# thu-uav/Multi-UAV-pursuit-evasion

Hardware: AMD Instinct MI355X
Metric: env agent-steps/sec at 65536 envs, HideAndSeek 3v1; 1/2/4/8 GPU (higher is better)
Workload: dtype f32

## Files before the change

multi-uav-pursuit-evasion_amd/csrc/hns_common.h:

```cpp
#pragma once
#include <hip/hip_runtime.h>

#include <cstdint>

#include "hns_device.h"

namespace hns {

constexpr int kEPB = 64;
constexpr int kMaxK = 4;
constexpr int kWideK = 16;
__host__ __device__ constexpr int red_stride(int NT) { return NT == 2 ? 11 : 9; }
enum { R_AERR = 0, R_TD, R_DIST, R_SPEED, R_CC, R_CD, R_CW, R_COLL,
       R_SMOOTH = R_AERR, R_FLAGS = R_TD,
       R_FX = R_DIST, R_FY = R_SPEED, R_FZ = R_CC,
       R_TWX = R_CD,
       R_F1X = 8,
       R_CPOS = R_DIST, R_CVEL = R_DIST + 3 };
enum { F_CAP = 1, F_BLOCKED = 2, F_DET = 4, F_DET1 = 8 };
constexpr int kGridStride = 516;
constexpr int kSmallWgPerCu = 2;
constexpr int kMaxT = 2;

template <int A>
struct Geo {
    static constexpr int NA = kEPB * A;
    static constexpr int T = kEPB * (A + 1);
};

struct Params {
    hns_cfg cfg;
    hns_buffers buf;
    const float *action;
    const uint8_t *reset_mask;
    uint32_t seed_lo, seed_hi, epoch;
    unsigned long long *prof;
    uint32_t cyl_magic;
    float *tasks;
    int32_t task_first;
    uint32_t prio_boost;
};

struct StepArgs {
    const float *action;
    float *prev_action, *drone_state, *pid_integ, *pid_last_rate, *throttle;
    const void *aux;
    const Params *rest;
};
static_assert(sizeof(StepArgs) == 64, "the argument block of the step kernel is sized for the fast launch path");
#define HNS_STEP_PARAMS                                                                                                                    \
    const Params *ka_rest, const float *ka_action, float *ka_prev_action, float *ka_drone_state, const void *ka_aux, float *ka_pid_integ, \
        float *ka_pid_last_rate, float *ka_throttle
#define HNS_STEP_ARGS_PACK const StepArgs ka{ka_action, ka_prev_action, ka_drone_state, ka_pid_integ, ka_pid_last_rate, ka_throttle, ka_aux, ka_rest}

HNS_DEV void warm_params(const Params *rest) {
    typedef const uint32_t __attribute__((address_space(4))) WordC;
    WordC *w = (WordC *)rest;
    uint32_t acc = 0;
#pragma unroll
    for (int i = 0; i < (int)((sizeof(Params) + 63) / 64); ++i) acc |= w[i * 16];
    asm volatile("" : : "s"(acc));
}

constexpr int kProfSlots = 16;
HNS_DEV void prof_mark(unsigned long long *prof, int slot) {
    if (prof && (threadIdx.x & 63) == 0) {
        int wave = blockIdx.x * (blockDim.x >> 6) + (threadIdx.x >> 6);
        prof[(size_t)wave * kProfSlots + slot] = (slot >= 14) ? __builtin_amdgcn_s_memrealtime() : __builtin_readcyclecounter();
#ifdef HNS_PROF_HWID
        if (slot == 0) prof[(size_t)wave * kProfSlots + 13] = __builtin_amdgcn_s_getreg(63492);
#endif
    }
}

struct Lds {
    int ds, cyl, cyl_stride, tp, red, ocyl, total;
};
__host__ __device__ inline int slab_floats(int A, int K, int NT);
__host__ __device__ inline int r4(int n) { return (n + 3) & ~3; }
__host__ __device__ constexpr int slab_rows(int A) { return A > 4 ? 32 : 64; }
__host__ __device__ inline int slab_floats(int A, int K, int NT) {
    const int rows = slab_rows(A);
    int m = rows * (NT == 2 ? 24 : HNS_SELF_DIM);
    if (K > kMaxK) K = 0;
    if (rows * K * 5 > m) m = rows * K * 5;
    if (rows * (A - 1) * 3 > m) m = rows * (A - 1) * 3;
    return r4(m);
}
__host__ __device__ inline Lds lds_layout(int A, int C, int K, int NT = 1) {
    Lds L;
    int o = 0;
    L.ds = o;    o += r4(kEPB * A * 13);
    L.cyl_stride = (3 * C) | 1;
    L.cyl = o;   o += r4(kEPB * L.cyl_stride);
    L.tp = o;    o += r4(kEPB * 3 * NT);
    L.red = o;   o += r4(kEPB * A * red_stride(NT));
    const int rows = K > kMaxK ? 0 : kEPB * A * K * 5, slabs = A * slab_floats(A, K, NT);
    L.ocyl = o;  o += r4(rows > slabs ? rows : slabs);
    L.total = o;
    return L;
}

template <int T>
HNS_DEV void coop_g2s(float *__restrict__ dst, const float *__restrict__ src, int n) {
    const int n4 = ((reinterpret_cast<uintptr_t>(src) & 15) == 0) ? (n >> 2) : 0;
    const float4 *s4 = reinterpret_cast<const float4 *>(src);
    float4 *d4 = reinterpret_cast<float4 *>(dst);
    for (int i = threadIdx.x; i < n4; i += T) d4[i] = s4[i];
    for (int i = (n4 << 2) + threadIdx.x; i < n; i += T) dst[i] = src[i];
}
template <int T>
HNS_DEV void coop_s2g(float *__restrict__ dst, const float *__restrict__ src, int n) {
    const int n4 = ((reinterpret_cast<uintptr_t>(dst) & 15) == 0) ? (n >> 2) : 0;
    const float4 *s4 = reinterpret_cast<const float4 *>(src);
    float4 *d4 = reinterpret_cast<float4 *>(dst);
    for (int i = threadIdx.x; i < n4; i += T) d4[i] = s4[i];
    for (int i = (n4 << 2) + threadIdx.x; i < n; i += T) dst[i] = src[i];
}
template <int T, int N>
HNS_DEV void coop_copy_full(float *__restrict__ dst, const float *__restrict__ src) {
    static_assert(N % 4 == 0, "float4 granularity");
    constexpr int N4 = N / 4;
    const float4 *s4 = reinterpret_cast<const float4 *>(src) + threadIdx.x;
    float4 *d4 = reinterpret_cast<float4 *>(dst) + threadIdx.x;
#pragma unroll
    for (int k = 0; k < (N4 + T - 1) / T; ++k)
        if (k * T + (int)threadIdx.x < N4) d4[k * T] = s4[k * T];
}
template <int T>
HNS_DEV void coop_s2g_masked(float *__restrict__ dst, const float *__restrict__ src, int n, int per_env,
                             const uint8_t *__restrict__ smask) {
    for (int i = threadIdx.x; i < n; i += T)
        if (smask[i / per_env]) dst[i] = src[i];
}
template <int T, bool TO_LDS>
HNS_DEV void coop_cyl(float *__restrict__ lds, float *__restrict__ g, int nenv, int c3, int stride, unsigned magic,
                      const uint8_t *__restrict__ smask) {
    for (int i = threadIdx.x; i < nenv * c3; i += T) {
        int le = (int)__umulhi((unsigned)i, magic), j = i - le * c3;
        if (TO_LDS) lds[le * stride + j] = g[i];
        else if (smask[le]) g[i] = lds[le * stride + j];
    }
}
HNS_DEV bool rigid_not_finite(const Rigid &s) {
    float a = s.pos.x;
    a = a + s.pos.y; a = a + s.pos.z; a = a + s.q.w; a = a + s.q.x; a = a + s.q.y; a = a + s.q.z;
    a = a + s.lin.x; a = a + s.lin.y; a = a + s.lin.z; a = a + s.ang.x; a = a + s.ang.y; a = a + s.ang.z;
    return (a - a) != 0.0f;
}
HNS_DEV void flag_nonfinite(uint32_t *word, bool bad, uint32_t bit) {
    if (word && bad) atomicOr(word, bit);
}
HNS_DEV void load_rigid(const float *r, Rigid &s) {
    s.pos = {r[0], r[1], r[2]};
    s.q = {r[3], r[4], r[5], r[6]};
    s.lin = {r[7], r[8], r[9]};
    s.ang = {r[10], r[11], r[12]};
}
HNS_DEV void store_rigid(float *r, const Rigid &s) {
    r[0] = s.pos.x; r[1] = s.pos.y; r[2] = s.pos.z;
    r[3] = s.q.w; r[4] = s.q.x; r[5] = s.q.y; r[6] = s.q.z;
    r[7] = s.lin.x; r[8] = s.lin.y; r[9] = s.lin.z;
    r[10] = s.ang.x; r[11] = s.ang.y; r[12] = s.ang.z;
}

HNS_DEV void st_f4(float4 *p, const float4 &v) {
    typedef float f4 __attribute__((ext_vector_type(4)));
    const f4 x = {v.x, v.y, v.z, v.w};
    asm volatile("global_store_dwordx4 %0, %1, off sc1\n\ts_nop 1" : : "v"(p), "v"(x) : "memory");
}
HNS_DEV void st_f1(float *p, float v) {
    asm volatile("global_store_dword %0, %1, off sc1\n\ts_nop 0" : : "v"(p), "v"(v) : "memory");
}

template <int NF, int ROWS = 64>
HNS_DEV void wave_store_rows(float *__restrict__ slab, float *__restrict__ gslice, const float (&row)[NF], int lane, int valid_rows = 64) {
    static_assert(ROWS == 64 || ROWS == 32, "whole wave or half a wave per pass");
    const uintptr_t gaddr = reinterpret_cast<uintptr_t>(gslice);
    const uintptr_t guni = ((uintptr_t)(uint32_t)__builtin_amdgcn_readfirstlane((int)(uint32_t)(gaddr >> 32)) << 32) |
                           (uintptr_t)(uint32_t)__builtin_amdgcn_readfirstlane((int)(uint32_t)gaddr);
    const int vrows = __builtin_amdgcn_readfirstlane(valid_rows);
#pragma unroll
    for (int half = 0; half < 64 / ROWS; ++half) {
        if (ROWS == 64 || (lane >> 5) == half) {
            float *mine = slab + (lane & (ROWS - 1)) * NF;
            if constexpr (NF % 4 == 0) {
#pragma unroll
                for (int i = 0; i < NF / 4; ++i) reinterpret_cast<float4 *>(mine)[i] = make_float4(row[4 * i], row[4 * i + 1], row[4 * i + 2], row[4 * i + 3]);
            } else if constexpr (NF % 2 == 0) {
#pragma unroll
                for (int i = 0; i < NF / 2; ++i) reinterpret_cast<float2 *>(mine)[i] = make_float2(row[2 * i], row[2 * i + 1]);
            } else {
#pragma unroll
                for (int i = 0; i < NF; ++i) mine[i] = row[i];
            }
        }
        __builtin_amdgcn_fence(__ATOMIC_RELEASE, "wavefront");
        __builtin_amdgcn_wave_barrier();
        constexpr int N4 = ROWS * NF / 4;
        const float4 *s4 = reinterpret_cast<const float4 *>(slab) + lane;
        typedef unsigned u4 __attribute__((ext_vector_type(4)));
        int rows_here = vrows - half * ROWS;
        rows_here = rows_here < 0 ? 0 : (rows_here > ROWS ? ROWS : rows_here);
        const __amdgpu_buffer_rsrc_t rs = __builtin_amdgcn_make_buffer_rsrc(reinterpret_cast<void *>(guni + (uintptr_t)half * ROWS * NF * 4), 0, rows_here * NF * 4, 0x00020000);
#pragma unroll
        for (int j = 0; j < (N4 + 63) / 64; ++j)
            if (j * 64 + lane < N4) {
                const float4 v = s4[j * 64];
                __builtin_amdgcn_raw_buffer_store_b128((u4){__float_as_uint(v.x), __float_as_uint(v.y), __float_as_uint(v.z), __float_as_uint(v.w)}, rs,
                                                       (j * 64 + lane) * 16, 0, 16 );
            }
        __builtin_amdgcn_fence(__ATOMIC_ACQUIRE, "wavefront");
        __builtin_amdgcn_wave_barrier();
    }
}

template <int NT, bool LOS, int KM = kMaxK, int KT = KM + 1, class Cfg>
HNS_DEV void cylinder_pass(const Cfg &c, int C, int K, const V3 &pos, const V3 &tp, const V3 &tpB, const float *cyl,
                           int bi[KM + 1], bool &any_block, bool &any_block1) {
    static_assert(KT >= 2 && KT <= KM + 1, "tracked keys");
    constexpr int kTrack = KT;
    uint32_t key[kTrack];
#pragma unroll
    for (int i = 0; i < kTrack; ++i) key[i] = 0x7F80000Fu;
    LosLine los = {}, los1 = {};
    if constexpr (LOS) los = d_los_setup(c, pos, tp);
    bool los_uncertain = false, los_uncertain1 = false;
    float mb0 = kInf, mt0 = kInf, mb1 = kInf, mt1 = kInf;
    any_block = false; any_block1 = false;
    if constexpr (LOS && NT == 2) los1 = d_los_setup(c, pos, tpB);
#pragma unroll 4
    for (int k = 0; k < C; ++k) {
        const float ccx = cyl[3 * k], ccy = cyl[3 * k + 1], ccz = cyl[3 * k + 2];
        const float ex = pos.x - ccx, ey = pos.y - ccy, ez = pos.z - ccz;
        if constexpr (LOS) any_block = d_los_cylinder_fast_acc(los, ccx, ccy, ccz, ex, ey, mb0, mt0) || any_block;
        if constexpr (LOS && NT == 2) any_block1 = d_los_cylinder_fast_acc(los1, ccx, ccy, ccz, ex, ey, mb1, mt1) || any_block1;
        const float d2 = HNS_FMA(ez, ez, HNS_FMA(ey, ey, ex * ex));
        uint32_t nk = (__float_as_uint(d2) & 0xFFFFFFF0u) | (uint32_t)k;
#pragma unroll
        for (int i = 0; i < kTrack; ++i) {
            uint32_t lo = min(key[i], nk);
            nk = max(key[i], nk);
            key[i] = lo;
        }
    }
    if constexpr (LOS) {
        los_uncertain = d_los_uncertain(los, mb0, mt0);
        if constexpr (NT == 2) los_uncertain1 = d_los_uncertain(los1, mb1, mt1);
        if (los_uncertain) any_block = d_blocked_exact(c, C, los, cyl);
        if (NT == 2 && los_uncertain1) any_block1 = d_blocked_exact(c, C, los1, cyl);
    }
    float bd[kTrack];
#pragma unroll
    for (int i = 0; i < kTrack; ++i) { bd[i] = __uint_as_float(key[i] & 0xFFFFFFF0u); bi[i] = (int)(key[i] & 15u); }
    bool order_safe = bd[0] > 1e-5f;
#pragma unroll
    for (int i = 0; i < kTrack - 1; ++i)
        if (i < K) order_safe = order_safe && (bd[i + 1] > bd[i] * 1.0000152587890625f);
    if (!order_safe) {
        if (!(__builtin_isfinite(pos.x) && __builtin_isfinite(pos.y) && __builtin_isfinite(pos.z))) {
#pragma unroll
            for (int i = 0; i < kTrack; ++i) bi[i] = i < C ? i : 0;
            return;
        }
#pragma unroll
        for (int i = 0; i < kTrack; ++i) { bd[i] = kInf; bi[i] = 0; }
        for (int k = 0; k < C; ++k) {
            float md = d_norm3(pos.x - cyl[3 * k], pos.y - cyl[3 * k + 1], pos.z - cyl[3 * k + 2]) - c.cylinder_size;
            if (md < bd[kTrack - 2]) {
                bd[kTrack - 2] = md; bi[kTrack - 2] = k;
#pragma unroll
                for (int i = kTrack - 2; i > 0; --i) {
                    if (bd[i] < bd[i - 1]) {
                        float td = bd[i]; bd[i] = bd[i - 1]; bd[i - 1] = td;
                        int ti = bi[i]; bi[i] = bi[i - 1]; bi[i - 1] = ti;
                    }
                }
            }
        }
    }
}

template <int A, int NT, bool STAGED = false, int PS = 13, int KM = kMaxK, class Cfg = hns_cfg>
HNS_DEV void agent_obs(const Cfg &c, int C, int K, int le, int a, const Rigid &s, const V3 &tp, const V3 &tpB, float progress,
                       const float *cyl, const float *sDS, float *gOth, float *sOCyl, float *gSelf, float *gState,
                       bool &blocked, bool &det, bool &blockedB, bool &detB, int knn_idx[KM], bool knn_masked[KM], bool st = true, bool st_oth = true,
                       float *gOCyl = nullptr, float *dist_out = nullptr, bool st_ocyl = true) {
    static_assert(!(STAGED && KM > kMaxK), "wide k-nearest selections are not staged");
    constexpr int SDW = NT == 2 ? 24 : HNS_SELF_DIM;
    const int lane = threadIdx.x & 63;
    float rtx = s.pos.x - tp.x, rty = s.pos.y - tp.y, rtz = s.pos.z - tp.z;
    float dist = d_norm3(rtx, rty, rtz);
    if (dist_out) *dist_out = dist;
    const float t = progress * c.inv_max_episode_length;
    V3 heading = d_quat_rot_x(s.q);
    V3 up = d_quat_rot_z(s.q, 1.0f);
    float4 v0 = make_float4(rtx, rty, rtz, s.q.w);
    float4 v1 = make_float4(s.q.x, s.q.y, s.q.z, s.lin.x);
    float4 v2 = make_float4(s.lin.y, s.lin.z, heading.x, heading.y);
    float4 v3 = make_float4(heading.z, up.x, up.y, up.z);
    float4 v4 = make_float4(t, t, t, t);
    float4 *so = reinterpret_cast<float4 *>(gSelf);
    if constexpr (!STAGED) {
        if (st) { so[0] = v0; so[1] = v1; so[2] = v2; so[3] = v3; so[4] = v4; }
        if (gState && st) {
            float4 *ss = reinterpret_cast<float4 *>(gState);
            ss[0] = v0; ss[1] = v1; ss[2] = v2; ss[3] = v3; ss[4] = v4;
        }
    }
    float dist1 = 0.0f;
    float4 v5 = make_float4(0, 0, 0, 0);
    if constexpr (NT == 2) {
        const float r1x = s.pos.x - tpB.x, r1y = s.pos.y - tpB.y, r1z = s.pos.z - tpB.z;
        dist1 = d_norm3(r1x, r1y, r1z);
        v5 = make_float4(r1x, r1y, r1z, 0.0f);
        if constexpr (!STAGED) {
            if (st) so[5] = v5;
            if (gState && st) reinterpret_cast<float4 *>(gState)[5] = v5;
        }
    }
    if constexpr (STAGED) {
        float row[SDW] = {v0.x, v0.y, v0.z, v0.w, v1.x, v1.y, v1.z, v1.w, v2.x, v2.y, v2.z, v2.w, v3.x, v3.y, v3.z, v3.w, v4.x, v4.y, v4.z, v4.w};
        if constexpr (NT == 2) { row[20] = v5.x; row[21] = v5.y; row[22] = v5.z; row[23] = v5.w; }
        if (st) wave_store_rows<SDW, slab_rows(A)>(sOCyl, gSelf - lane * SDW, row, lane);
        if (gState && st) wave_store_rows<SDW, slab_rows(A)>(sOCyl, gState - lane * SDW, row, lane);
    }
    if (A > 1) {
        float o[(A > 1 ? A - 1 : 1) * 3];
#pragma unroll
        for (int w = 0; w < A - 1; ++w) {
            const int j = w + (w >= a ? 1 : 0);
            const float *rj = sDS + (le * A + j) * PS;
            o[3 * w] = s.pos.x - rj[0]; o[3 * w + 1] = s.pos.y - rj[1]; o[3 * w + 2] = s.pos.z - rj[2];
        }
        if constexpr (STAGED) {
            if (st_oth) wave_store_rows<(A > 1 ? A - 1 : 1) * 3, slab_rows(A)>(sOCyl, gOth - lane * (A - 1) * 3, o, lane);
        } else if (!st_oth) {
        } else if ((((A - 1) * 3) & 1) == 0) {
            float2 *g2 = reinterpret_cast<float2 *>(gOth);
#pragma unroll
            for (int i = 0; i < (A - 1) * 3 / 2; ++i) g2[i] = make_float2(o[2 * i], o[2 * i + 1]);
        } else {
#pragma unroll
            for (int i = 0; i < (A - 1) * 3; ++i) gOth[i] = o[i];
        }
    }
    int bi[KM + 1];
    bool any_block, any_block1;
    cylinder_pass<NT, true, KM>(c, C, K, s.pos, tp, tpB, cyl, bi, any_block, any_block1);
    blocked = any_block;
    det = (dist < c.drone_detect_radius) && !blocked;
    if constexpr (NT == 2) {
        blockedB = any_block1;
        detB = (dist1 < c.drone_detect_radius) && !any_block1;
    }
    float *oc = KM > kMaxK ? gOCyl : sOCyl + (le * A + a) * K * 5;
    float krow[STAGED ? kMaxK * 5 : 1];
#pragma unroll
    for (int sidx = 0; sidx < KM; ++sidx) {
        if (sidx < K) {
            const float *cc = cyl + 3 * bi[sidx];
            bool masked = cc[2] < 0.0f;
            knn_idx[sidx] = bi[sidx];
            knn_masked[sidx] = masked;
            float *row = STAGED ? krow + sidx * 5 : oc + sidx * 5;
            const float mv = c.mask_value, ch = c.cylinder_height, cs = c.cylinder_size;
            row[0] = masked ? mv : s.pos.x - cc[0];
            row[1] = masked ? mv : s.pos.y - cc[1];
            row[2] = masked ? mv : s.pos.z - cc[2];
            row[3] = masked ? mv : ch;
            row[4] = masked ? mv : cs;
        }
    }
    if constexpr (STAGED) {
        if (st_ocyl) {
            if (K == 3) {
                float r[15];
#pragma unroll
                for (int i = 0; i < 15; ++i) r[i] = krow[i];
                wave_store_rows<15, slab_rows(A)>(sOCyl, gOCyl - lane * 15, r, lane);
            } else if (K == 4) {
                wave_store_rows<20, slab_rows(A)>(sOCyl, gOCyl - lane * 20, krow, lane);
            } else if (K == 2) {
                float r[10];
#pragma unroll
                for (int i = 0; i < 10; ++i) r[i] = krow[i];
                wave_store_rows<10, slab_rows(A)>(sOCyl, gOCyl - lane * 10, r, lane);
            } else {
                float r[5];
#pragma unroll
                for (int i = 0; i < 5; ++i) r[i] = krow[i];
                wave_store_rows<5, slab_rows(A)>(sOCyl, gOCyl - lane * 5, r, lane);
            }
        }
    }
}

}
```

multi-uav-pursuit-evasion_amd/csrc/hns_step_body.inc:

```
    HNS_STEP_ARGS_PACK;
    static_assert(GEN || KM == kMaxK, "wide k-nearest selections: the generic instantiation");
    static_assert(!MOTOR || GEN, "motor-command input: the generic instantiation");
    static_assert(CS == 0 || (!GEN && !PROF && CS <= HNS_MAX_CYLINDERS), "fixed shapes: the tuned instantiation only");
    typedef const Params __attribute__((address_space(4))) ParamsC;
    ParamsC &p = *(ParamsC *)ka.rest;
    constexpr int NA = Geo<A>::NA, SD = NT == 2 ? 24 : HNS_SELF_DIM, kRedS = red_stride(NT), T3 = 3 * NT;
    extern __shared__ __align__(16) float smem[];
    const auto &c = p.cfg;
    const auto &b = p.buf;
    const int tid = threadIdx.x, lane = tid & 63;
    const int e0 = blockIdx.x * kEPB;
    int nv = kEPB, Etot = 0;
    if constexpr (GEN) { Etot = c.num_envs; nv = Etot - e0 < kEPB ? Etot - e0 : kEPB; }
    if (tid < NA) {
        const int le = tid / A, a = tid - le * A;
        const unsigned ia = (unsigned)e0 * A + tid;
        const bool valid = !GEN || le < nv;
        const int vrows = GEN ? nv * A - (tid & ~63) : 64;
        const unsigned il = GEN ? (unsigned)(e0 + (le < nv ? le : nv - 1)) * A + a : ia;
        const float4 act4 = reinterpret_cast<const float4 *>(ka.action)[il];
        float4 prev4 = make_float4(0.f, 0.f, 0.f, 0.f);
        if constexpr (!MOTOR) prev4 = reinterpret_cast<const float4 *>(ka.prev_action)[il];
        constexpr int N4 = 64 * 13 / 4;
        const float4 *rows4 = reinterpret_cast<const float4 *>(ka.drone_state + ((size_t)e0 * A + (tid & ~63)) * 13) + lane;
        static_assert(N4 > 192 && N4 <= 256, "three full passes and a partial one");
        float4 rr0 = make_float4(0.f, 0.f, 0.f, 0.f), rr1 = rr0, rr2 = rr0, rr3 = rr0;
        if constexpr (!GEN) {
            rr0 = rows4[0]; rr1 = rows4[64]; rr2 = rows4[128];
            if (lane < N4 - 192) rr3 = rows4[192];
        }
        float4 integ4 = make_float4(0.f, 0.f, 0.f, 0.f);
        if constexpr (NT == 1 && !MOTOR) integ4 = reinterpret_cast<const float4 *>(ka.pid_integ)[il];
        float4 last4 = make_float4(0.f, 0.f, 0.f, 0.f);
        if constexpr (MOTOR) last4.w = ka.pid_last_rate[(size_t)il * 4 + 3];
        else last4 = reinterpret_cast<const float4 *>(ka.pid_last_rate)[il];
        unsigned rp = 0;
        if constexpr (NT == 1) {
            const uint8_t *rpp = static_cast<const uint8_t *>(ka.aux);
            const uint8_t *rsafe = rpp ? rpp : reinterpret_cast<const uint8_t *>(ka.action);
            const unsigned byte = rsafe[GEN ? (e0 + (le < nv ? le : nv - 1)) : (e0 + le)];
            rp = rpp ? byte : 0u;
        }
        float4 thr4 = reinterpret_cast<const float4 *>(ka.throttle)[il];
        constexpr int kStage = NT == 2 ? (3 * HNS_MAX_CYLINDERS + A - 1) / A : 1, kOwnCyl = NT == 2 ? (HNS_MAX_CYLINDERS + A - 1) / A : 1;
        float stage_v[kStage], own_c[kOwnCyl][3];
        if constexpr (NT == 2) {
            const uintptr_t cw = reinterpret_cast<uintptr_t>(ka.aux);
            const int Cq = CS ? CS : (int)(cw & 15) + 1;
            typedef const float __attribute__((address_space(1))) gcf;
            const gcf *cyl0 = reinterpret_cast<const gcf *>(cw & ~(uintptr_t)15);
            const gcf *gc = cyl0 + (size_t)e0 * Cq * 3 + lane;
#pragma unroll
            for (int i = 0; i < kStage; ++i) {
                const int pass = (tid >> 6) + i * A;
                stage_v[i] = (pass < 3 * Cq && (!GEN || pass * 64 + lane < nv * 3 * Cq)) ? gc[pass * 64] : 0.0f;
            }
            const gcf *gcy = cyl0 + (size_t)(e0 + (GEN && le >= nv ? nv - 1 : le)) * Cq * 3;
#pragma unroll
            for (int i = 0; i < kOwnCyl; ++i) {
                const int k = a + i * A;
                const int kc = k < Cq ? k : 0;
                own_c[i][0] = gcy[3 * kc]; own_c[i][1] = gcy[3 * kc + 1]; own_c[i][2] = gcy[3 * kc + 2];
            }
            if constexpr (!MOTOR) integ4 = reinterpret_cast<const float4 *>(ka.pid_integ)[il];
        }
        __builtin_amdgcn_sched_barrier(0);
        if constexpr (PROF) prof_mark(p.prof, 0);
        if constexpr (PROF) prof_mark(p.prof, 14);
        const int C = CS ? CS : c.num_cylinders, K = CS ? 3 : c.obs_max_cylinder;
        const bool with_state = c.write_critic_state && b.state_drones != nullptr;
        const LdsV3 L = lds_layout_v3(A, C, K, NT);
        float *sPub = smem + L.pub, *sCyl = smem + L.cyl, *sTp = smem + L.tp, *sRed = smem + L.red;
        float *slab = smem + L.slab + (tid >> 6) * L.slab_stride;
        V3 etp0 = {0.f, 0.f, 0.f}, etp1 = {0.f, 0.f, 0.f};
        if constexpr (NT == 2) {
            {
                const uint8_t *rsafe = b.reset_pid ? b.reset_pid : reinterpret_cast<const uint8_t *>(ka.action);
                const unsigned byte = rsafe[e0 + (GEN && le >= nv ? nv - 1 : le)];
                rp = b.reset_pid ? byte : 0u;
            }
            const float *gt = b.target_pos + (size_t)(e0 + (GEN && le >= nv ? nv - 1 : le)) * T3;
            etp0 = V3{gt[0], gt[1], gt[2]};
            etp1 = V3{gt[3], gt[4], gt[5]};
        }
        float4 ta = act4;
        if constexpr (!MOTOR) ta = d_action_tanh(act4);
        Rigid s;
        if constexpr (GEN) {
            load_rigid(ka.drone_state + (size_t)il * 13, s);
        } else {
            float4 *s4 = reinterpret_cast<float4 *>(slab) + lane;
            s4[0] = rr0; s4[64] = rr1; s4[128] = rr2;
            if (lane < N4 - 192) s4[192] = rr3;
            __builtin_amdgcn_fence(__ATOMIC_RELEASE, "wavefront");
            __builtin_amdgcn_wave_barrier();
            load_rigid(slab + lane * 13, s);
            __builtin_amdgcn_fence(__ATOMIC_ACQUIRE, "wavefront");
            __builtin_amdgcn_wave_barrier();
        }
        if constexpr (PROF) prof_mark(p.prof, 1);
        const bool boost = p.prio_boost != 0;
        if (boost) __builtin_amdgcn_s_setprio(1);
        const float los_t = last4.w;
        float cmd[4], thr_diff, aerr, thrust[4], moment[4];
        float ctbr4[4], trate[3];
        if constexpr (MOTOR) {
            cmd[0] = ta.x; cmd[1] = ta.y; cmd[2] = ta.z; cmd[3] = ta.w;
            aerr = b.action_error[il];
        } else {
        {
            const bool r = rp != 0;
            integ4.x = r ? 0.0f : integ4.x; integ4.y = r ? 0.0f : integ4.y; integ4.z = r ? 0.0f : integ4.z;
            last4.x = r ? 0.0f : last4.x; last4.y = r ? 0.0f : last4.y; last4.z = r ? 0.0f : last4.z;
        }
        d_ctbr_pid_squashed(c, ta, s.q, s.ang, prev4, integ4, last4, cmd, aerr, ctbr4, trate);
        asm volatile("" : "+v"(thr4.x), "+v"(thr4.y), "+v"(thr4.z), "+v"(thr4.w));
        if (b.ctbr && valid) reinterpret_cast<float4 *>(b.ctbr)[ia] = make_float4(ctbr4[0], ctbr4[1], ctbr4[2], ctbr4[3]);
        if (b.target_rate && valid) reinterpret_cast<float4 *>(b.target_rate)[ia] = make_float4(trate[0], trate[1], trate[2], 0.0f);
        }
        d_rotor(c, cmd, thr4, thrust, moment, thr_diff);
        const float ts = ((thrust[0] + thrust[1]) + thrust[2]) + thrust[3];
        const V3 tw = d_quat_rot_z(s.q, ts);
        const float inv_ntw = d_downwash_inv_norm(tw);
        {
            float *pub = sPub + tid * kPub;
            pub[0] = s.pos.x; pub[1] = s.pos.y; pub[2] = s.pos.z;
            pub[3] = tw.x; pub[4] = tw.y; pub[5] = tw.z;
            pub[9] = inv_ntw;
            pub[10] = los_t;
            float *red = sRed + tid * kRedS;
            red[R_AERR] = aerr; red[R_TD] = thr_diff;
            if constexpr (NT == 2) {
                const int los = (int)los_t;
                const V3 f0 = d_prey_pursuer_term(c, s.pos, etp0, (los & 1) != 0);
                const V3 f1 = d_prey_pursuer_term(c, s.pos, etp1, (los & 2) != 0);
                red[R_FX] = f0.x; red[R_FY] = f0.y; red[R_FZ] = f0.z;
                red[R_F1X] = f1.x; red[R_F1X + 1] = f1.y; red[R_F1X + 2] = f1.z;
                float *term = smem + L.term + le * L.term_stride;
#pragma unroll
                for (int i = 0; i < kOwnCyl; ++i) {
                    const int k = a + i * A;
                    if (k < C) {
                        float tx, ty;
                        d_prey_cylinder_term(c, etp1, own_c[i][0], own_c[i][1], own_c[i][2], tx, ty);
                        term[2 * k] = tx; term[2 * k + 1] = ty;
                    }
                }
                const int c3 = 3 * C;
#pragma unroll
                for (int i = 0; i < kStage; ++i) {
                    const int pass = (tid >> 6) + i * A;
                    if (pass < c3) {
                        const int idx = pass * 64 + lane;
                        const int row = (int)__umulhi((unsigned)idx, p.cyl_magic), col = idx - row * c3;
                        sCyl[row * L.cyl_stride + col] = stage_v[i];
                    }
                }
            }
        }
        if constexpr (PROF) prof_mark(p.prof, 2);
        __syncthreads();
        if constexpr (PROF) prof_mark(p.prof, 12);
        V3 fdw = {0.f, 0.f, 0.f};
#pragma unroll
        for (int o = 0; o < A - 1; ++o) {
            const int j = o + (o >= a ? 1 : 0);
            const float *pj = sPub + (le * A + j) * kPub;
            const V3 posj = {pj[0], pj[1], pj[2]}, twj = {pj[3], pj[4], pj[5]};
            const V3 fj = d_downwash_pair(s.pos, posj, twj, pj[9]);
            fdw.x = (o == 0) ? fj.x : fdw.x + fj.x;
            fdw.y = (o == 0) ? fj.y : fdw.y + fj.y;
            fdw.z = (o == 0) ? fj.z : fdw.z + fj.z;
        }
        const V3 fw = {tw.x + fdw.x, tw.y + fdw.y, tw.z + fdw.z};
        V3 tb;
        tb.x = ((c.rotor_py[0] * thrust[0] + c.rotor_py[1] * thrust[1]) + c.rotor_py[2] * thrust[2]) + c.rotor_py[3] * thrust[3];
        tb.y = -(((c.rotor_px[0] * thrust[0] + c.rotor_px[1] * thrust[1]) + c.rotor_px[2] * thrust[2]) + c.rotor_px[3] * thrust[3]);
        tb.z = ((moment[0] + moment[1]) + moment[2]) + moment[3];
        d_integrate(c, s, fw, tb);
        if constexpr (CONTACT) {
            float *red = sRed + tid * kRedS;
            red[R_CPOS] = s.pos.x; red[R_CPOS + 1] = s.pos.y; red[R_CPOS + 2] = s.pos.z;
            red[R_CVEL] = s.lin.x; red[R_CVEL + 1] = s.lin.y; red[R_CVEL + 2] = s.lin.z;
        } else {
            flag_nonfinite(b.nonfinite, valid && rigid_not_finite(s), 1u);
            float *pub = sPub + tid * kPub;
            pub[6] = s.pos.x; pub[7] = s.pos.y; pub[8] = s.pos.z;
        }
        if (valid) {
            st_f4(reinterpret_cast<float4 *>(b.throttle) + ia, thr4);
            if constexpr (!MOTOR) {
                st_f4(reinterpret_cast<float4 *>(b.pid_integ) + ia, integ4);
                st_f4(reinterpret_cast<float4 *>(b.prev_action) + ia, prev4);
                st_f1(b.action_error + ia, aerr);
            }
        }
        if constexpr (CONTACT) {
            __syncthreads();
            const float *cyl = sCyl + le * L.cyl_stride;
            d_contact_step<A, CS>(c, s, a, sRed + le * A * kRedS, cyl, C);
            flag_nonfinite(b.nonfinite, valid && rigid_not_finite(s), 1u);
            float *pub = sPub + tid * kPub;
            pub[6] = s.pos.x; pub[7] = s.pos.y; pub[8] = s.pos.z;
        }
        {
            const float row[13] = {s.pos.x, s.pos.y, s.pos.z, s.q.w, s.q.x, s.q.y, s.q.z, s.lin.x, s.lin.y, s.lin.z, s.ang.x, s.ang.y, s.ang.z};
            wave_store_rows<13>(slab, b.drone_state + ((size_t)e0 * A + (tid & ~63)) * 13, row, lane, vrows);
        }
        if constexpr (PROF) prof_mark(p.prof, 3);
        __syncthreads();
        if constexpr (PROF) prof_mark(p.prof, 8);
        if (boost) __builtin_amdgcn_s_setprio(0);
        const float progress = sTp[kEPB * T3 + le];
        const V3 tp = {sTp[le * T3], sTp[le * T3 + 1], sTp[le * T3 + 2]};
        V3 tpB = tp;
        if constexpr (NT == 2) tpB = V3{sTp[le * T3 + 3], sTp[le * T3 + 4], sTp[le * T3 + 5]};
        const float *cyl = sCyl + le * L.cyl_stride;
        const float rtx = s.pos.x - tp.x, rty = s.pos.y - tp.y, rtz = s.pos.z - tp.z;
        const float d = d_norm3(rtx, rty, rtz);
        int knn_idx[KM + 1];
        bool knn_masked[KM];
        bool blocked, blockedB;
        cylinder_pass<NT, true, KM, (CS ? 4 : KM + 1)>(c, C, K, s.pos, tp, tpB, cyl, knn_idx, blocked, blockedB);
        const bool det = (d < c.drone_detect_radius) && !blocked;
        last4.w = (float)((blocked ? 1 : 0) + (NT == 2 && blockedB ? 2 : 0));
        if constexpr (MOTOR) { if (valid) b.pid_last_rate[(size_t)ia * 4 + 3] = last4.w; }
        else if (valid) reinterpret_cast<float4 *>(b.pid_last_rate)[ia] = last4;
#pragma unroll
        for (int sidx = 0; sidx < KM; ++sidx) knn_masked[sidx] = (sidx < K) ? cyl[3 * knn_idx[sidx] + 2] < 0.0f : false;
        if constexpr (PROF) prof_mark(p.prof, 9);
        bool cap_ok = (d < c.catch_radius) && !blocked, all_blk = blocked, detB = false;
        float dn = d;
        float r1x = 0.f, r1y = 0.f, r1z = 0.f;
        if constexpr (NT == 2) {
            r1x = s.pos.x - tpB.x; r1y = s.pos.y - tpB.y; r1z = s.pos.z - tpB.z;
            const float d1 = d_norm3(r1x, r1y, r1z);
            detB = (d1 < c.drone_detect_radius) && !blockedB;
            cap_ok = cap_ok || ((d1 < c.catch_radius) && !blockedB);
            all_blk = blocked && blockedB;
            dn = d1 < d ? d1 : d;
        }
        const float act = (dn > c.catch_radius) ? 1.0f : 0.0f;
        const float dist_rew = (-c.dist_reward_coef * dn) * act;
        bool fast = false;
        {
            const float sp2 = HNS_FMA(s.lin.z, s.lin.z, HNS_FMA(s.lin.y, s.lin.y, s.lin.x * s.lin.x));
            const float v2 = c.v_drone * c.v_drone;
            fast = sp2 > v2 * 1.00000190734863f;
            if (!fast && !(sp2 < v2 * 0.99999809265137f)) fast = __builtin_sqrtf(sp2) > c.v_drone;
        }
        const float speed_rew = -c.speed_coef * (fast ? 1.0f : 0.0f);
        float cc = 0.f, cd = 0.f;
        const float rc = c.cylinder_size + c.collision_radius, rc2 = rc * rc;
#pragma unroll
        for (int sidx = 0; sidx < KM; ++sidx) {
            if (sidx < K) {
                const float *cy = cyl + 3 * knn_idx[sidx];
                const float rx = s.pos.x - cy[0], ry = s.pos.y - cy[1];
                const float s2 = HNS_FMA(ry, ry, rx * rx);
                bool h = s2 < rc2 * 0.99999618530273f;
                if (!h && !(s2 > rc2 * 1.00000381469727f)) h = (__builtin_sqrtf(s2) - c.cylinder_size) < c.collision_radius;
                float hit = h ? 1.0f : 0.0f;
                if (knn_masked[sidx]) hit = 0.0f;
                cc = (sidx == 0) ? hit : cc + hit;
            }
        }
        float cr = -c.collision_coef * cc;
        const float dd2 = c.coll_drone_dist * c.coll_drone_dist;
#pragma unroll
        for (int o = 0; o < A - 1; ++o) {
            const int j = o + (o >= a ? 1 : 0);
            const float *rj = sPub + (le * A + j) * kPub + 6;
            const float ex = s.pos.x - rj[0], ey = s.pos.y - rj[1], ez = s.pos.z - rj[2];
            const float s3 = HNS_FMA(ez, ez, HNS_FMA(ey, ey, ex * ex));
            bool h = s3 < dd2 * 0.99999809265137f;
            if (!h && !(s3 > dd2 * 1.00000190734863f)) h = __builtin_sqrtf(s3) < c.coll_drone_dist;
            const float hit = h ? 1.0f : 0.0f;
            cd = (o == 0) ? hit : cd + hit;
        }
        cr = cr + -c.collision_coef * cd;
        const float cw = ((s.pos.z > c.max_height) ? 1.0f : 0.0f) + ((HNS_FMA(s.pos.y, s.pos.y, s.pos.x * s.pos.x) > c.arena_sq) ? 1.0f : 0.0f);
        cr = cr + -c.collision_coef * cw;
        float sm = 0.0f;
        if (c.use_deployment) sm = c.smoothness_coef * d_expf(-aerr);
        {
            float *red = sRed + tid * kRedS;
            red[R_DIST] = dist_rew; red[R_SPEED] = speed_rew; red[R_CC] = cc; red[R_CD] = cd; red[R_CW] = cw;
            red[R_COLL] = cr; red[R_SMOOTH] = sm;
            red[R_FLAGS] = __int_as_float((cap_ok ? F_CAP : 0) | (all_blk ? F_BLOCKED : 0) | (det ? F_DET : 0) | (detB ? F_DET1 : 0));
        }
        if constexpr (PROF) prof_mark(p.prof, 4);
        __syncthreads();
        if constexpr (PROF) prof_mark(p.prof, 5);
        bool det_any = false, det_any1 = false;
#pragma unroll
        for (int j = 0; j < A; ++j) {
            const int fl = __float_as_int(sRed[(le * A + j) * kRedS + R_FLAGS]);
            det_any |= (fl & F_DET) != 0;
            det_any1 |= (fl & F_DET1) != 0;
        }
        {
            const float t = progress * c.inv_max_episode_length;
            const V3 heading = d_quat_rot_x(s.q), up = d_quat_rot_z(s.q, 1.0f);
            const float m = c.mask_value;
            float row[SD] = {det_any ? rtx : m, det_any ? rty : m, det_any ? rtz : m, s.q.w, s.q.x, s.q.y, s.q.z, s.lin.x, s.lin.y, s.lin.z,
                             heading.x, heading.y, heading.z, up.x, up.y, up.z, t, t, t, t};
            if constexpr (NT == 2) { row[20] = det_any1 ? r1x : m; row[21] = det_any1 ? r1y : m; row[22] = det_any1 ? r1z : m; row[23] = 0.0f; }
            wave_store_rows<SD, slab_rows_v4(A, NT)>(slab, b.obs_self + ((size_t)e0 * A + (tid & ~63)) * SD, row, lane, vrows);
            if (with_state) {
                float rs[SD];
#pragma unroll
                for (int i = 0; i < SD; ++i) rs[i] = row[i];
                rs[0] = rtx; rs[1] = rty; rs[2] = rtz;
                if constexpr (NT == 2) { rs[20] = r1x; rs[21] = r1y; rs[22] = r1z; }
                wave_store_rows<SD, slab_rows_v4(A, NT)>(slab, b.state_drones + ((size_t)e0 * A + (tid & ~63)) * SD, rs, lane, vrows);
            }
        }
        if constexpr (A > 1) {
            float o[(A > 1 ? A - 1 : 1) * 3];
#pragma unroll
            for (int w = 0; w < A - 1; ++w) {
                const int j = w + (w >= a ? 1 : 0);
                const float *rj = sPub + (le * A + j) * kPub + 6;
                o[3 * w] = s.pos.x - rj[0]; o[3 * w + 1] = s.pos.y - rj[1]; o[3 * w + 2] = s.pos.z - rj[2];
            }
            wave_store_rows<(A > 1 ? A - 1 : 1) * 3, slab_rows_v4(A, NT)>(slab, b.obs_others + ((size_t)e0 * A + (tid & ~63)) * (A - 1) * 3, o, lane, vrows);
        }
        if constexpr (KM > kMaxK) {
            const float mv = c.mask_value, ch = c.cylinder_height, cs = c.cylinder_size;
            float *oc = b.obs_cylinders + (size_t)ia * K * 5;
            if (valid) {
#pragma unroll
                for (int sidx = 0; sidx < KM; ++sidx) {
                    if (sidx < K) {
                        const float *cc = cyl + 3 * knn_idx[sidx];
                        const bool masked = knn_masked[sidx];
                        oc[sidx * 5] = masked ? mv : s.pos.x - cc[0];
                        oc[sidx * 5 + 1] = masked ? mv : s.pos.y - cc[1];
                        oc[sidx * 5 + 2] = masked ? mv : s.pos.z - cc[2];
                        oc[sidx * 5 + 3] = masked ? mv : ch;
                        oc[sidx * 5 + 4] = masked ? mv : cs;
                    }
                }
            }
        } else {
            float krow[kMaxK * 5];
            const float mv = c.mask_value, ch = c.cylinder_height, cs = c.cylinder_size;
#pragma unroll
            for (int sidx = 0; sidx < kMaxK; ++sidx) {
                const float *cc = cyl + 3 * ((sidx < K) ? knn_idx[sidx] : 0);
                const bool masked = knn_masked[sidx];
                const float rx = s.pos.x - cc[0], ry = s.pos.y - cc[1], rz = s.pos.z - cc[2];
                krow[sidx * 5] = masked ? mv : rx;
                krow[sidx * 5 + 1] = masked ? mv : ry;
                krow[sidx * 5 + 2] = masked ? mv : rz;
                krow[sidx * 5 + 3] = masked ? mv : ch;
                krow[sidx * 5 + 4] = masked ? mv : cs;
            }
            float *g = b.obs_cylinders + ((size_t)e0 * A + (tid & ~63)) * K * 5;
            if (K == 3) {
                float r[15];
#pragma unroll
                for (int i = 0; i < 15; ++i) r[i] = krow[i];
                wave_store_rows<15, slab_rows_v4(A, NT)>(slab, g, r, lane, vrows);
            } else if (K == 4) {
                wave_store_rows<20, slab_rows_v4(A, NT)>(slab, g, krow, lane, vrows);
            } else if (K == 2) {
                float r[10];
#pragma unroll
                for (int i = 0; i < 10; ++i) r[i] = krow[i];
                wave_store_rows<10, slab_rows_v4(A, NT)>(slab, g, r, lane, vrows);
            } else {
                float r[5];
#pragma unroll
                for (int i = 0; i < 5; ++i) r[i] = krow[i];
                wave_store_rows<5, slab_rows_v4(A, NT)>(slab, g, r, lane, vrows);
            }
        }
        if constexpr (PROF) prof_mark(p.prof, 6);
    } else {
        __builtin_amdgcn_s_setprio(2);
        const int le = lane;
        const bool valid = !GEN || le < nv;
        const int e = e0 + (valid ? le : nv - 1);
#ifndef HNS_NO_WARM
        warm_params(ka.rest);
#endif
        if constexpr (PROF) prof_mark(p.prof, 0);
        if constexpr (PROF) prof_mark(p.prof, 14);
        const int C = CS ? CS : c.num_cylinders, K = CS ? 3 : c.obs_max_cylinder, E = c.stats_stride;
        const LdsV3 L = lds_layout_v3(A, C, K, NT);
        float *sPub = smem + L.pub, *sCyl = smem + L.cyl, *sTp = smem + L.tp, *sRed = smem + L.red, *sEnvOut = smem + L.envout;
        float *cylw = sCyl + le * L.cyl_stride;
        const float *gt = b.target_pos + (size_t)e * T3;
        const V3 tp0 = {gt[0], gt[1], gt[2]};
        V3 tp1 = tp0;
        if constexpr (NT == 2) tp1 = V3{gt[3], gt[4], gt[5]};
        float progress = b.progress[e];
        if constexpr (NT == 1 && GEN) {
            const float *gr = b.cylinders + (size_t)e * C * 3;
            for (int j = 0; j < 3 * C; ++j) cylw[j] = gr[j];
            __builtin_amdgcn_fence(__ATOMIC_RELEASE, "wavefront");
            __builtin_amdgcn_wave_barrier();
        } else if constexpr (NT == 1) {
            const float *gc = b.cylinders + (size_t)e0 * C * 3 + lane;
            const int c3 = 3 * C;
            int i0 = 0;
            for (; i0 + 24 <= c3; i0 += 24) {
                float cv[24];
#pragma unroll
                for (int i = 0; i < 24; ++i) cv[i] = gc[(i0 + i) * 64];
#pragma unroll
                for (int i = 0; i < 24; ++i) {
                    const int idx = (i0 + i) * 64 + lane;
                    const int row = (int)__umulhi((unsigned)idx, p.cyl_magic), col = idx - row * c3;
                    sCyl[row * L.cyl_stride + col] = cv[i];
                }
            }
            for (; i0 < c3; i0 += 3) {
                float cv[3];
#pragma unroll
                for (int i = 0; i < 3; ++i) cv[i] = gc[(i0 + i) * 64];
#pragma unroll
                for (int i = 0; i < 3; ++i) {
                    const int idx = (i0 + i) * 64 + lane;
                    const int row = (int)__umulhi((unsigned)idx, p.cyl_magic), col = idx - row * c3;
                    sCyl[row * L.cyl_stride + col] = cv[i];
                }
            }
            __builtin_amdgcn_fence(__ATOMIC_RELEASE, "wavefront");
            __builtin_amdgcn_wave_barrier();
        }
        progress += 1.0f;
        sTp[kEPB * T3 + le] = progress;
        if constexpr (PROF) prof_mark(p.prof, 1);
        float st[HNS_NUM_STATS];
        if constexpr (NT == 1) {
#pragma unroll
            for (int i = 0; i < HNS_NUM_STATS; ++i) st[i] = b.stats[(size_t)i * E + e];
        }
        bool out_of_arena = false;
        const V3 Fenv = d_prey_arena_term(c, tp0, out_of_arena);
        float fcx = 0.f, fcy = 0.f;
        if constexpr (NT == 2) {
            const float *cylg = b.cylinders + (size_t)e * C * 3;
            if ((C & 3) == 0) {
                const float4 *g4 = reinterpret_cast<const float4 *>(cylg);
                for (int k0 = 0; k0 < C; k0 += 4) {
                    const float4 q0 = g4[3 * (k0 >> 2)], q1 = g4[3 * (k0 >> 2) + 1], q2 = g4[3 * (k0 >> 2) + 2];
                    const float v[12] = {q0.x, q0.y, q0.z, q0.w, q1.x, q1.y, q1.z, q1.w, q2.x, q2.y, q2.z, q2.w};
#pragma unroll
                    for (int i = 0; i < 4; ++i) {
                        float tx, ty;
                        d_prey_cylinder_term(c, tp0, v[3 * i], v[3 * i + 1], v[3 * i + 2], tx, ty);
                        fcx += tx;
                        fcy += ty;
                    }
                }
            } else {
                for (int k = 0; k < C; ++k) {
                    float tx, ty;
                    d_prey_cylinder_term(c, tp0, cylg[3 * k], cylg[3 * k + 1], cylg[3 * k + 2], tx, ty);
                    fcx += tx;
                    fcy += ty;
                }
            }
        } else {
#pragma unroll 4
            for (int k = 0; k < C; ++k) {
                float tx, ty;
                d_prey_cylinder_term(c, tp0, cylw[3 * k], cylw[3 * k + 1], cylw[3 * k + 2], tx, ty);
                fcx += tx;
                fcy += ty;
            }
        }
        V3 Fenv1 = {0.f, 0.f, 0.f};
        float gcx = 0.f, gcy = 0.f;
        if constexpr (NT == 2) {
            bool out1 = false;
            Fenv1 = d_prey_arena_term(c, tp1, out1);
            out_of_arena = out_of_arena || out1;
#pragma unroll
            for (int i = 0; i < HNS_NUM_STATS; ++i) st[i] = b.stats[(size_t)i * E + e];
        }
        if constexpr (PROF) prof_mark(p.prof, 2);
        __syncthreads();
        if constexpr (PROF) prof_mark(p.prof, 12);
#ifndef HNS_NO_PIN
#pragma unroll
        for (int i = 0; i < HNS_NUM_STATS; ++i) asm volatile("" : "+v"(st[i]));
#endif
        V3 F = {0.f, 0.f, 0.f}, G = {0.f, 0.f, 0.f};
#pragma unroll
        for (int j = 0; j < A; ++j) {
            if constexpr (NT == 2) {
                const float *red = sRed + (le * A + j) * kRedS;
                F.x = (j == 0) ? red[R_FX] : F.x + red[R_FX];
                F.y = (j == 0) ? red[R_FY] : F.y + red[R_FY];
                F.z = (j == 0) ? red[R_FZ] : F.z + red[R_FZ];
                G.x = (j == 0) ? red[R_F1X] : G.x + red[R_F1X];
                G.y = (j == 0) ? red[R_F1X + 1] : G.y + red[R_F1X + 1];
                G.z = (j == 0) ? red[R_F1X + 2] : G.z + red[R_F1X + 2];
            } else {
                const float *pj = sPub + (le * A + j) * kPub;
                const V3 dp = {pj[0], pj[1], pj[2]};
                const int los = (int)pj[10];
                const V3 fp = d_prey_pursuer_term(c, dp, tp0, (los & 1) != 0);
                F.x = (j == 0) ? fp.x : F.x + fp.x;
                F.y = (j == 0) ? fp.y : F.y + fp.y;
                F.z = (j == 0) ? fp.z : F.z + fp.z;
            }
        }
        if constexpr (NT == 2) {
            const float *term = smem + L.term + le * L.term_stride;
#pragma unroll 4
            for (int k = 0; k < C; ++k) {
                gcx += term[2 * k];
                gcy += term[2 * k + 1];
            }
        }
        F.x = F.x + Fenv.x; F.y = F.y + Fenv.y; F.z = F.z + Fenv.z;
        F.x = F.x + fcx; F.y = F.y + fcy; F.z = F.z + 0.0f;
        const V3 tvel = {(c.v_prey * F.x) / (__builtin_fabsf(F.x) + 1e-5f), (c.v_prey * F.y) / (__builtin_fabsf(F.y) + 1e-5f),
                         (c.v_prey * F.z) / (__builtin_fabsf(F.z) + 1e-5f)};
        V3 tpn = {tp0.x + tvel.x * c.dt, tp0.y + tvel.y * c.dt, tp0.z + tvel.z * c.dt};
        if constexpr (CONTACT) {
            float vx = 0.0f, vy = 0.0f;
            d_contact_cylinders<false, CS>(tpn, vx, vy, cylw, C, c.contact_rt, c.contact_rt2, c.cylinder_height);
        }
        sTp[le * T3] = tpn.x; sTp[le * T3 + 1] = tpn.y; sTp[le * T3 + 2] = tpn.z;
        { const float sf = (tpn.x + tpn.y) + tpn.z; flag_nonfinite(b.nonfinite, valid && (sf - sf) != 0.0f, 2u); }
        V3 tvel1 = {0.f, 0.f, 0.f};
        if constexpr (NT == 2) {
            G.x = G.x + Fenv1.x; G.y = G.y + Fenv1.y; G.z = G.z + Fenv1.z;
            G.x = G.x + gcx; G.y = G.y + gcy; G.z = G.z + 0.0f;
            tvel1 = V3{(c.v_prey * G.x) / (__builtin_fabsf(G.x) + 1e-5f), (c.v_prey * G.y) / (__builtin_fabsf(G.y) + 1e-5f),
                       (c.v_prey * G.z) / (__builtin_fabsf(G.z) + 1e-5f)};
            const V3 tpn1 = {tp1.x + tvel1.x * c.dt, tp1.y + tvel1.y * c.dt, tp1.z + tvel1.z * c.dt};
            sTp[le * T3 + 3] = tpn1.x; sTp[le * T3 + 4] = tpn1.y; sTp[le * T3 + 5] = tpn1.z;
            { const float sf = (tpn1.x + tpn1.y) + tpn1.z; flag_nonfinite(b.nonfinite, valid && (sf - sf) != 0.0f, 2u); }
        }
        {
            sEnvOut[le * T3] = tvel.x; sEnvOut[le * T3 + 1] = tvel.y; sEnvOut[le * T3 + 2] = tvel.z;
            if constexpr (NT == 2) { sEnvOut[le * T3 + 3] = tvel1.x; sEnvOut[le * T3 + 4] = tvel1.y; sEnvOut[le * T3 + 5] = tvel1.z; }
            env_store_slice<GEN>(sTp, b.target_pos + (size_t)e0 * T3, kEPB * T3, lane, nv * T3);
            env_store_slice<GEN>(sEnvOut, b.target_vel + (size_t)e0 * T3, kEPB * T3, lane, nv * T3);
        }
        if constexpr (CONTACT) __syncthreads();
        {
            float sum_ae = 0.f, sum_td = 0.f, max_td = 0.f;
#pragma unroll
            for (int j = 0; j < A; ++j) {
                const float *red = sRed + (le * A + j) * kRedS;
                const float td = red[R_TD];
                sum_ae = (j == 0) ? red[R_AERR] : sum_ae + red[R_AERR];
                sum_td = (j == 0) ? td : sum_td + td;
                max_td = (j == 0) ? td : (td > max_td ? td : max_td);
            }
            const float mae = sum_ae * c.inv_num_agents;
            st[HNS_ST_ACTION_ERROR_ORDER1_MEAN] += mae;
            if (mae > st[HNS_ST_ACTION_ERROR_ORDER1_MAX]) st[HNS_ST_ACTION_ERROR_ORDER1_MAX] = mae;
            st[HNS_ST_OUT_OF_ARENA] = ((st[HNS_ST_OUT_OF_ARENA] != 0.0f) || out_of_arena) ? 1.0f : 0.0f;
            st[HNS_ST_SMOOTHNESS_COEF] = c.smoothness_coef;
            st[HNS_ST_SMOOTHNESS_MEAN] += sum_td * c.inv_num_agents;
            if (max_td > st[HNS_ST_SMOOTHNESS_MAX]) st[HNS_ST_SMOOTHNESS_MAX] = max_td;
        }
        if constexpr (PROF) prof_mark(p.prof, 3);
        __syncthreads();
        if constexpr (PROF) prof_mark(p.prof, 8);
        if constexpr (PROF) prof_mark(p.prof, 4);
        __syncthreads();
        if constexpr (PROF) prof_mark(p.prof, 5);
        const float iA = c.inv_num_agents;
        bool any_cap = false, all_blocked = true, any_coll = false, det_any = false, det_any1 = false;
        float sum_dist = 0, sum_speed = 0, sum_cc = 0, sum_cd = 0, sum_cw = 0, sum_coll = 0, sum_smooth = 0;
#pragma unroll
        for (int j = 0; j < A; ++j) {
            const float *red = sRed + (le * A + j) * kRedS;
            const int fl = __float_as_int(red[R_FLAGS]);
            any_cap |= (fl & F_CAP) != 0;
            all_blocked &= (fl & F_BLOCKED) != 0;
            det_any |= (fl & F_DET) != 0;
            det_any1 |= (fl & F_DET1) != 0;
            any_coll |= red[R_COLL] < 0.0f;
            if (j == 0) {
                sum_dist = red[R_DIST]; sum_speed = red[R_SPEED]; sum_cc = red[R_CC]; sum_cd = red[R_CD]; sum_cw = red[R_CW];
                sum_coll = red[R_COLL]; sum_smooth = red[R_SMOOTH];
            } else {
                sum_dist += red[R_DIST]; sum_speed += red[R_SPEED]; sum_cc += red[R_CC]; sum_cd += red[R_CD]; sum_cw += red[R_CW];
                sum_coll += red[R_COLL]; sum_smooth += red[R_SMOOTH];
            }
        }
        const float detf = (det_any || (NT == 2 && det_any1)) ? 1.0f : 0.0f;
        const float detect_rew = c.detect_reward_coef * detf;
        const float catch_rew = c.catch_reward_coef * (any_cap ? 1.0f : 0.0f);
        float sum_rew = 0.f;
#pragma unroll
        for (int j = 0; j < A; ++j) {
            const float *red = sRed + (le * A + j) * kRedS;
            const float r = ((((red[R_DIST] + detect_rew) + catch_rew) + red[R_COLL]) + red[R_SPEED]) + red[R_SMOOTH];
            sEnvOut[le * A + j] = r;
            sum_rew = (j == 0) ? r : sum_rew + r;
        }
        env_store_slice<GEN>(sEnvOut, b.reward + (size_t)e0 * A, kEPB * A, lane, nv * A);
        flag_nonfinite(b.nonfinite, valid && (sum_rew - sum_rew) != 0.0f, 4u);
#define ST(i) st[i]
        ST(HNS_ST_DISTANCE_REWARD) += sum_dist * iA;
        ST(HNS_ST_SUM_DETECT_STEP) += 1.0f * detf;
        float sdet = detect_rew, scat = catch_rew;
#pragma unroll
        for (int j = 1; j < A; ++j) { sdet += detect_rew; scat += catch_rew; }
        ST(HNS_ST_DETECT_REWARD) += sdet * iA;
        const bool capture_flag = catch_rew != 0.0f;
        ST(HNS_ST_BLOCKED) += all_blocked ? 1.0f : 0.0f;
        ST(HNS_ST_SUCCESS) = (capture_flag || ST(HNS_ST_SUCCESS) != 0.0f) ? 1.0f : 0.0f;
        const float cur = (capture_flag ? 1.0f : 0.0f) * progress + (capture_flag ? 0.0f : 1.0f) * (float)c.max_episode_length;
        if (cur < ST(HNS_ST_FIRST_CAPTURE_STEP)) ST(HNS_ST_FIRST_CAPTURE_STEP) = cur;
        ST(HNS_ST_CATCH_REWARD) += scat * iA;
        ST(HNS_ST_SPEED_REWARD) += sum_speed * iA;
        ST(HNS_ST_COLLISION_CYLINDER) += sum_cc * iA;
        ST(HNS_ST_COLLISION_DRONE) += sum_cd * iA;
        ST(HNS_ST_COLLISION) += any_coll ? 1.0f : 0.0f;
        ST(HNS_ST_COLLISION_WALL) += sum_cw * iA;
        ST(HNS_ST_COLLISION_REWARD) += sum_coll * iA;
        ST(HNS_ST_SMOOTHNESS_REWARD) += sum_smooth * iA;
        const bool done = progress >= (float)c.max_episode_length;
        if (done) {
            ST(HNS_ST_COLLISION) = ST(HNS_ST_COLLISION) / progress;
            ST(HNS_ST_ACTION_ERROR_ORDER1_MEAN) = ST(HNS_ST_ACTION_ERROR_ORDER1_MEAN) / progress;
            ST(HNS_ST_TARGET_PREDICTED_ERROR) = ST(HNS_ST_TARGET_PREDICTED_ERROR) / progress;
            ST(HNS_ST_SMOOTHNESS_MEAN) = ST(HNS_ST_SMOOTHNESS_MEAN) / progress;
            ST(HNS_ST_SMOOTHNESS_REWARD) = ST(HNS_ST_SMOOTHNESS_REWARD) / progress;
            ST(HNS_ST_DISTANCE_REWARD) = ST(HNS_ST_DISTANCE_REWARD) / progress;
            ST(HNS_ST_DETECT_REWARD) = ST(HNS_ST_DETECT_REWARD) / progress;
            ST(HNS_ST_CATCH_REWARD) = ST(HNS_ST_CATCH_REWARD) / progress;
            ST(HNS_ST_COLLISION_REWARD) = ST(HNS_ST_COLLISION_REWARD) / progress;
            ST(HNS_ST_COLLISION_WALL) = ST(HNS_ST_COLLISION_WALL) / progress;
            ST(HNS_ST_COLLISION_DRONE) = ST(HNS_ST_COLLISION_DRONE) / progress;
            ST(HNS_ST_COLLISION_CYLINDER) = ST(HNS_ST_COLLISION_CYLINDER) / progress;
            ST(HNS_ST_SPEED_REWARD) = ST(HNS_ST_SPEED_REWARD) / progress;
        }
        ST(HNS_ST_RETURN) += sum_rew * iA;
#undef ST
        if (valid) {
            b.done[e] = (uint8_t)done;
            if (b.detect) b.detect[e] = (uint8_t)((det_any ? 1 : 0) | (NT == 2 && det_any1 ? 2 : 0));
            b.progress[e] = progress;
#pragma unroll
            for (int i = 0; i < HNS_NUM_STATS; ++i) st_f1(b.stats + (size_t)i * E + e, st[i]);
        }
        if constexpr (PROF) prof_mark(p.prof, 6);
    }
    if constexpr (PROF) prof_mark(p.prof, 7);
    if constexpr (PROF) prof_mark(p.prof, 15);
```

Measured before the change: 10.75 billion.

## Skip unchanged per-env stat row loads and stores using wave ballots

Per-env stats are now classified. Rows that are never written are not loaded or stored. The done-only row is loaded and stored only when some env in the wave finishes. Rows that rarely change are stored only when the wave ballot shows at least one lane changed. Early-finalized smoothness and action-error stats, plus progress, are stored before the second barrier so their stores overlap the remaining work. This cuts global memory traffic in a store-heavy kernel, at the cost of extra ballots, register pressure for the saved copies, and a reliance on the never-written rows staying constant.

```diff
diff --git a/multi-uav-pursuit-evasion_amd/csrc/hns_common.h b/multi-uav-pursuit-evasion_amd/csrc/hns_common.h
--- a/multi-uav-pursuit-evasion_amd/csrc/hns_common.h
+++ b/multi-uav-pursuit-evasion_amd/csrc/hns_common.h
@@ -171,6 +171,22 @@
 }
 HNS_DEV void st_f1(float *p, float v) {
     asm volatile("global_store_dword %0, %1, off sc1\n\ts_nop 0" : : "v"(p), "v"(v) : "memory");
+}
+
+constexpr bool stat_never(int i) { return i == HNS_ST_DISTANCE_PREDICTED_REWARD || i == HNS_ST_DISTANCE_THRESHOLD_L; }
+constexpr bool stat_done_only(int i) { return i == HNS_ST_TARGET_PREDICTED_ERROR; }
+constexpr bool stat_early(int i) {
+    return i == HNS_ST_ACTION_ERROR_ORDER1_MEAN || i == HNS_ST_ACTION_ERROR_ORDER1_MAX || i == HNS_ST_OUT_OF_ARENA || i == HNS_ST_SMOOTHNESS_COEF ||
+           i == HNS_ST_SMOOTHNESS_MEAN || i == HNS_ST_SMOOTHNESS_MAX;
+}
+constexpr bool stat_voted(int i) {
+    return i == HNS_ST_SUCCESS || i == HNS_ST_SPEED_REWARD || i == HNS_ST_COLLISION_CYLINDER || i == HNS_ST_COLLISION_DRONE || i == HNS_ST_DETECT_REWARD ||
+           i == HNS_ST_CATCH_REWARD || i == HNS_ST_SMOOTHNESS_REWARD || i == HNS_ST_SMOOTHNESS_MAX || i == HNS_ST_FIRST_CAPTURE_STEP ||
+           i == HNS_ST_ACTION_ERROR_ORDER1_MAX || i == HNS_ST_OUT_OF_ARENA || i == HNS_ST_SMOOTHNESS_COEF || stat_done_only(i);
+}
+HNS_DEV void store_stat_row(int row, float *p, float now, float was, bool valid) {
+    if (stat_voted(row) && __builtin_amdgcn_ballot_w64(valid && __float_as_int(now) != __float_as_int(was)) == 0) return;
+    if (valid) st_f1(p, now);
 }
 
 template <int NF, int ROWS = 64>
diff --git a/multi-uav-pursuit-evasion_amd/csrc/hns_step_body.inc b/multi-uav-pursuit-evasion_amd/csrc/hns_step_body.inc
--- a/multi-uav-pursuit-evasion_amd/csrc/hns_step_body.inc
+++ b/multi-uav-pursuit-evasion_amd/csrc/hns_step_body.inc
@@ -434,11 +434,16 @@
         progress += 1.0f;
         sTp[kEPB * T3 + le] = progress;
         if constexpr (PROF) prof_mark(p.prof, 1);
-        float st[HNS_NUM_STATS];
-        if constexpr (NT == 1) {
-#pragma unroll
-            for (int i = 0; i < HNS_NUM_STATS; ++i) st[i] = b.stats[(size_t)i * E + e];
-        }
+        const bool done = progress >= (float)c.max_episode_length;
+        const bool any_done = __builtin_amdgcn_ballot_w64(done) != 0;
+        float st[HNS_NUM_STATS] = {};
+        auto load_stats = [&]() {
+#pragma unroll
+            for (int i = 0; i < HNS_NUM_STATS; ++i)
+                if (!stat_never(i) && !stat_done_only(i)) st[i] = b.stats[(size_t)i * E + e];
+            if (any_done) st[HNS_ST_TARGET_PREDICTED_ERROR] = b.stats[(size_t)HNS_ST_TARGET_PREDICTED_ERROR * E + e];
+        };
+        if constexpr (NT == 1) load_stats();
         bool out_of_arena = false;
         const V3 Fenv = d_prey_arena_term(c, tp0, out_of_arena);
         float fcx = 0.f, fcy = 0.f;
@@ -480,16 +485,19 @@
             bool out1 = false;
             Fenv1 = d_prey_arena_term(c, tp1, out1);
             out_of_arena = out_of_arena || out1;
-#pragma unroll
-            for (int i = 0; i < HNS_NUM_STATS; ++i) st[i] = b.stats[(size_t)i * E + e];
+            load_stats();
         }
         if constexpr (PROF) prof_mark(p.prof, 2);
         __syncthreads();
         if constexpr (PROF) prof_mark(p.prof, 12);
 #ifndef HNS_NO_PIN
 #pragma unroll
-        for (int i = 0; i < HNS_NUM_STATS; ++i) asm volatile("" : "+v"(st[i]));
+        for (int i = 0; i < HNS_NUM_STATS; ++i)
+            if (!stat_never(i)) asm volatile("" : "+v"(st[i]));
 #endif
+        float was[HNS_NUM_STATS];
+#pragma unroll
+        for (int i = 0; i < HNS_NUM_STATS; ++i) was[i] = st[i];
         V3 F = {0.f, 0.f, 0.f}, G = {0.f, 0.f, 0.f};
 #pragma unroll
         for (int j = 0; j < A; ++j) {
@@ -564,6 +572,14 @@
             st[HNS_ST_SMOOTHNESS_COEF] = c.smoothness_coef;
             st[HNS_ST_SMOOTHNESS_MEAN] += sum_td * c.inv_num_agents;
             if (max_td > st[HNS_ST_SMOOTHNESS_MAX]) st[HNS_ST_SMOOTHNESS_MAX] = max_td;
+            if (done) {
+                st[HNS_ST_ACTION_ERROR_ORDER1_MEAN] = st[HNS_ST_ACTION_ERROR_ORDER1_MEAN] / progress;
+                st[HNS_ST_SMOOTHNESS_MEAN] = st[HNS_ST_SMOOTHNESS_MEAN] / progress;
+            }
+#pragma unroll
+            for (int i = 0; i < HNS_NUM_STATS; ++i)
+                if (stat_early(i)) store_stat_row(i, b.stats + (size_t)i * E + e, st[i], was[i], valid);
+            if (valid) b.progress[e] = progress;
         }
         if constexpr (PROF) prof_mark(p.prof, 3);
         __syncthreads();
@@ -624,12 +640,9 @@
         ST(HNS_ST_COLLISION_WALL) += sum_cw * iA;
         ST(HNS_ST_COLLISION_REWARD) += sum_coll * iA;
         ST(HNS_ST_SMOOTHNESS_REWARD) += sum_smooth * iA;
-        const bool done = progress >= (float)c.max_episode_length;
         if (done) {
             ST(HNS_ST_COLLISION) = ST(HNS_ST_COLLISION) / progress;
-            ST(HNS_ST_ACTION_ERROR_ORDER1_MEAN) = ST(HNS_ST_ACTION_ERROR_ORDER1_MEAN) / progress;
             ST(HNS_ST_TARGET_PREDICTED_ERROR) = ST(HNS_ST_TARGET_PREDICTED_ERROR) / progress;
-            ST(HNS_ST_SMOOTHNESS_MEAN) = ST(HNS_ST_SMOOTHNESS_MEAN) / progress;
             ST(HNS_ST_SMOOTHNESS_REWARD) = ST(HNS_ST_SMOOTHNESS_REWARD) / progress;
             ST(HNS_ST_DISTANCE_REWARD) = ST(HNS_ST_DISTANCE_REWARD) / progress;
             ST(HNS_ST_DETECT_REWARD) = ST(HNS_ST_DETECT_REWARD) / progress;
@@ -645,10 +658,12 @@
         if (valid) {
             b.done[e] = (uint8_t)done;
             if (b.detect) b.detect[e] = (uint8_t)((det_any ? 1 : 0) | (NT == 2 && det_any1 ? 2 : 0));
-            b.progress[e] = progress;
-#pragma unroll
-            for (int i = 0; i < HNS_NUM_STATS; ++i) st_f1(b.stats + (size_t)i * E + e, st[i]);
-        }
+        }
+#pragma unroll
+        for (int i = 0; i < HNS_NUM_STATS; ++i)
+            if (!stat_never(i) && !stat_early(i) && !stat_done_only(i)) store_stat_row(i, b.stats + (size_t)i * E + e, st[i], was[i], valid);
+        if (any_done) store_stat_row(HNS_ST_TARGET_PREDICTED_ERROR, b.stats + (size_t)HNS_ST_TARGET_PREDICTED_ERROR * E + e, st[HNS_ST_TARGET_PREDICTED_ERROR],
+                                     was[HNS_ST_TARGET_PREDICTED_ERROR], valid);
         if constexpr (PROF) prof_mark(p.prof, 6);
     }
     if constexpr (PROF) prof_mark(p.prof, 7);
```

Result: no change. 10.70 billion (-0.5%).
